# crlotwhite/pytorch_hmm

Hardware: AMD Instinct MI355X
Metric: frames/sec forward-backward+Viterbi, B=32 T=2000 N=128, 1/2/4/8 GPU (higher is better)
Workload: dtype f32; 1 GPU; HMMPyTorch forward_backward + viterbi_decode; batch_per_gpu=32, global_batch=32, seq_len=2000, num_states=128, transition=left_to_right(0.7), world_size_seen=1, parallelism=batch-sharded x1, streams=2, gather=False, hip_graph=False, step_pipelining=per-op streams, no per-step join, transition_plan=True, fb_kernel=chains + posterior followers in one launch, viterbi_kernel=chains + log leaders + decode followers in one launch

## Files before the change

pytorch_hmm_amd/csrc/recur.h:

```cpp
#pragma once
#include "band.h"
#include "common.h"
#include "logcr.h"
#include "post.h"

namespace hmm355 {

enum RecKind : int { kFbAlpha = 0, kFbBeta = 1, kVit = 2 };
typedef unsigned int u32x2_t __attribute__((__vector_size__(2 * sizeof(unsigned int))));

#ifndef HMM355_EMIS_AHEAD_ALPHA
#define HMM355_EMIS_AHEAD_ALPHA 1
#endif
#ifndef HMM355_EMIS_AHEAD_BETA
#define HMM355_EMIS_AHEAD_BETA 2
#endif
#ifndef HMM355_EMIS_AHEAD_VIT
#define HMM355_EMIS_AHEAD_VIT 2
#endif
constexpr int emis_ahead(int kind) {
  return kind == kFbAlpha ? HMM355_EMIS_AHEAD_ALPHA : kind == kFbBeta ? HMM355_EMIS_AHEAD_BETA : HMM355_EMIS_AHEAD_VIT;
}
#ifdef HMM355_RED_FORM
#define HMM355_RED_FORM_ALPHA HMM355_RED_FORM
#define HMM355_RED_FORM_BETA HMM355_RED_FORM
#define HMM355_RED_FORM_VIT HMM355_RED_FORM
#endif
#ifndef HMM355_RED_FORM_ALPHA
#define HMM355_RED_FORM_ALPHA 1
#endif
#ifndef HMM355_RED_FORM_BETA
#define HMM355_RED_FORM_BETA 3
#endif
#ifndef HMM355_RED_FORM_VIT
#define HMM355_RED_FORM_VIT 3
#endif
constexpr int red_form(int kind) {
  return kind == kFbAlpha ? HMM355_RED_FORM_ALPHA : kind == kFbBeta ? HMM355_RED_FORM_BETA : HMM355_RED_FORM_VIT;
}

constexpr int kStampWaves = 512 * 16;
static __device__ unsigned long long g_rec_stamps[kStamp ? kStampWaves * 8 : 1];
constexpr bool kStampItems = HMM355_STAMP > 1;

template <int NP>
struct RC {
  static constexpr int NW = NP / 16;
  static constexpr int NT = NW * kWave;
  static constexpr int NBLK = NP / 64;
  static constexpr int RING = 64;
  static constexpr int OFF_PART = 0;
  static constexpr int OFF_EMIS = OFF_PART + 2 * NP * 2;
  static constexpr int OFF_RING = OFF_EMIS + 3 * 16 * NP;
  static constexpr int OFF_SC = OFF_RING + RING * NP;
  static constexpr int OFF_M = OFF_SC + RING * 64;
  static constexpr int MRING = 128;
  static constexpr int OFF_LOGT = OFF_M + MRING;
  static constexpr int LDS_FLOATS = OFF_LOGT + 512;
  static_assert(LDS_FLOATS * 4 <= kExclusiveLds, "LDS layout too large");
  static constexpr int OFF_LEFT = LDS_FLOATS;
  static_assert((OFF_LEFT + 16) * 4 <= kExclusiveLds, "end-row LDS layout too large");
  static constexpr int PSR = 64;
  static constexpr int OFF_PSR = LDS_FLOATS;
  static_assert((OFF_PSR + PSR * NP / 4) * 4 <= kExclusiveLds, "fused Viterbi LDS layout too large");
};

template <int NP>
struct kRbHelpers {
  static constexpr int NH = NP <= 128 ? RC<NP>::NW / 2 : 0;
  static constexpr int NT = RC<NP>::NT + NH * kWave;
  static_assert(NH <= 8, "kProgSlots");
};
template <int NP>
constexpr int kFbNT = kRbHelpers<NP>::NT;

namespace red {
constexpr int kA = 1, kB = 2;
constexpr int stages(int F) { return 6 - (F & kA ? 1 : 0) - (F & kB ? 1 : 0); }
constexpr bool triple_at(int F, int L) { return (L == 0 && (F & kA)) || (L == 2 && (F & kB)); }
constexpr int level(int F, int S) {
  int L = 0;
  for (int s = 0; s < S; ++s) L += triple_at(F, L) ? 2 : 1;
  return L;
}
}
template <bool MAX, int SHR>
__device__ __forceinline__ float red_shr(float acc, float src) {
  const float o = __builtin_bit_cast(
      float, __builtin_amdgcn_update_dpp(0, __builtin_bit_cast(int, src), 0x110 + SHR, 0xF, 0xF, true));
  return MAX ? fmaxf(acc, o) : acc + o;
}
#define HMM355_RED_SHR2(VOL, OP)                                                            \
  asm VOL(OP " %0, %1, %0 row_shr:%2 row_mask:0xf bank_mask:0xf bound_ctrl:1\n\t"           \
          OP " %0, %1, %0 row_shr:%3 row_mask:0xf bank_mask:0xf bound_ctrl:1"               \
          : "+v"(acc) : "v"(src), "n"(S2), "n"(S3))
template <bool MAX, int S2, int S3, bool PIN>
__device__ __forceinline__ float red_shr2_asm(float acc, float src) {
  if constexpr (MAX && PIN) HMM355_RED_SHR2(volatile, "v_max_f32_dpp");
  else if constexpr (MAX) HMM355_RED_SHR2(, "v_max_f32_dpp");
  else if constexpr (PIN) HMM355_RED_SHR2(volatile, "v_add_f32_dpp");
  else HMM355_RED_SHR2(, "v_add_f32_dpp");
  return acc;
}
#undef HMM355_RED_SHR2
template <bool MAX, int S, int F = 0, bool PIN = false>
__device__ __forceinline__ float wave_red_level(float x) {
  constexpr int L = red::level(F, S);
  if constexpr (red::triple_at(F, L)) {
    constexpr int K = L == 0 ? 1 : 4;
    return red_shr2_asm<MAX, 2 * K, 3 * K, PIN>(red_shr<MAX, K>(x, x), x);
  } else {
    constexpr int CTRL = L == 0 ? 0xB1 : L == 1 ? 0x4E : L == 2 ? 0x124 : L == 3 ? 0x128 : L == 4 ? 0x142 : 0x143;
    const float o = __builtin_bit_cast(
        float, __builtin_amdgcn_update_dpp(0, __builtin_bit_cast(int, x), CTRL, 0xF, 0xF, L >= 4));
    return MAX ? fmaxf(x, o) : x + o;
  }
}
__device__ __forceinline__ float wave_lane63(float x) {
  return __builtin_bit_cast(float, __builtin_amdgcn_readlane(__builtin_bit_cast(int, x), 63));
}

template <int F = 0>
__device__ __forceinline__ float wave_sum_bcast(float x) {
  static_for<0, red::stages(F)>([&](auto S) { x = wave_red_level<false, decltype(S)::value, F>(x); });
  return wave_lane63(x);
}
template <int F = 0>
__device__ __forceinline__ float wave_max_bcast(float x) {
  static_for<0, red::stages(F)>([&](auto S) { x = wave_red_level<true, decltype(S)::value, F>(x); });
  return wave_lane63(x);
}

constexpr int fill_gaps(int F) { return red::stages(F) + 2; }
constexpr int fill_slots(int F, int G) { return G == fill_gaps(F) - 2 ? 1 : 2; }
constexpr int emis_wait_gap(int F) {
#ifdef HMM355_EMIS_WAIT_GAP
  return HMM355_EMIS_WAIT_GAP;
#else
  return F == 0 ? 4 : red::stages(F) - 1;
#endif
}
constexpr int fill_cnt(int G, int NU, int F = 0) {
  const int NG = fill_gaps(F);
  int rem = NU, all = 0;
  for (int i = 0; i < NG; ++i) all += fill_slots(F, i);
  for (int i = 0; i < NG; ++i) {
    const int g = i == 0 ? NG - 1 : i - 1;
    const int c = fill_slots(F, g) < rem ? fill_slots(F, g) : rem;
    if (g == G) return c + (G == NG - 1 && NU > all ? NU - all : 0);
    rem -= c;
  }
  return 0;
}
constexpr int fill_lo(int G, int NU, int F = 0) {
  int lo = 0;
  for (int g = 0; g < G; ++g) lo += fill_cnt(g, NU, F);
  return lo;
}
__device__ __forceinline__ void fill_pin(float& x) { asm volatile("" : "+v"(x)); }
template <bool MAX, int F = 0, typename FILL>
__device__ __forceinline__ float wave_red_fill(float x, FILL&& fill) {
  constexpr int NS = red::stages(F);
  static_for<0, NS>([&](auto S) {
    __builtin_amdgcn_sched_barrier(0);
    fill(S);
    __builtin_amdgcn_sched_barrier(0);
    x = wave_red_level<MAX, decltype(S)::value, F, true>(x);
    if constexpr (!red::triple_at(F, red::level(F, decltype(S)::value))) fill_pin(x);
  });
  __builtin_amdgcn_sched_barrier(0);
  fill(std::integral_constant<int, NS>{});
  __builtin_amdgcn_sched_barrier(0);
  x = wave_lane63(x);
  __builtin_amdgcn_sched_barrier(0);
  fill(std::integral_constant<int, NS + 1>{});
  __builtin_amdgcn_sched_barrier(0);
  return x;
}

#if HMM355_RED_PROBE
static __global__ void red_probe_kernel(const float* in, float* out, int n) {
  const int v = blockIdx.x * (blockDim.x / kWave) + threadIdx.x / kWave;
  if (v >= n) return;
  const float x = in[(size_t)v * kWave + (threadIdx.x & (kWave - 1))];
  static_for<0, 4>([&](auto F) {
    const float m = wave_max_bcast<decltype(F)::value>(x), s = wave_sum_bcast<decltype(F)::value>(x);
    if ((threadIdx.x & (kWave - 1)) == 0) {
      out[(size_t)v * 8 + decltype(F)::value] = m;
      out[(size_t)v * 8 + 4 + decltype(F)::value] = s;
    }
  });
}
#endif

template <int NB>
__device__ __forceinline__ void prods(const float (&p)[NB], const float (&e)[NB], float (&prod)[NB]) {
// ... 677 lines not shown
  constexpr bool FB = KIND != kVit;
  constexpr int NM = NP / 64;
  typedef float f2 __attribute__((ext_vector_type(2)));
  const int tid = threadIdx.x;
  if (tid >= C::NT) {
    rec_rb_helper<NP, KIND>(a, lds, b);
    return;
  }
  __builtin_amdgcn_s_setprio(2);
  const int w = tid >> 6, l = tid & 63, r = l >> 4, c = l & 15;
  const int g = 4 * w + r;
  const int x = c >> 2;
  const int o = 4 * g + x;
  const int T = a.T, N = a.N;
  float* ring = lds + C::OFF_RING;
  float* Pv = lds + C::OFF_PART;

  f2 Mk[4][NM][2];
#pragma unroll
  for (int k = 0; k < 4; ++k)
#pragma unroll
    for (int m = 0; m < NM; ++m)
#pragma unroll
      for (int e = 0; e < 4; ++e) {
        const int i = 64 * m + 4 * c + e, ok = 4 * g + (k ^ x);
        const bool in = i < N && ok < N;
        const size_t idx = in ? (KIND == kFbBeta ? (size_t)ok * N + i : (size_t)i * N + ok) : 0;
        const float v = a.mat[idx];
        Mk[k][m][e >> 1][e & 1] = FB ? __expf(in ? v : -INFINITY) : (in ? v : -INFINITY);
      }

  const int qend = T;
  const int nblocks = (qend + 15) / 16;
  {
    float er0[5];
    if (KIND == kVit) rec_logt_fill<NP>(lds, l);
    rec_load<NP, KIND>(a, b, 0, w, l, er0);
    rec_stage<NP, KIND>(a, lds, 0, w, l, er0);
  }
  lds_barrier();

  auto emis = [&](int rho, int idx) -> const float& { return rec_emis<NP>(lds, rho, idx); };
  const bool writer = (c & 3) == 0;
  {
    const float v0 = rec_row0<NP, KIND>(a, b, o, emis(0, o));
    if (writer) {
      ring[o] = v0;
      if (KIND == kFbBeta) Pv[o] = v0 * emis(0, o);
    }
  }
  lds_barrier();

  RecStamps stamps;
  stamps.begin();
  auto mark = [&](int k) { stamps.mark(k); };

  auto stepq = [&](int q) {
    if (kStamp) mark(3);
    const float* src = KIND == kFbBeta ? Pv + ((q - 1) & 1) * NP : ring + ((q - 1) & (C::RING - 1)) * NP;
    float eo = emis(q, o);
    f2 yin[NM][2];
#pragma unroll
    for (int m = 0; m < NM; ++m) {
      const float4 v4 = *reinterpret_cast<const float4*>(src + 64 * m + 4 * c);
      yin[m][0] = f2{v4.x, v4.y};
      yin[m][1] = f2{v4.z, v4.w};
    }
    keep(eo);
    if (kStamp) { keep(yin[0][0]); mark(0); }
    float s0, s1, s2, s3;
    float cs = 0.f;
    if (FB) {
      f2 acc[4];
#pragma unroll
      for (int k = 0; k < 4; ++k) acc[k] = f2{0.f, 0.f};
      f2 ysum = f2{0.f, 0.f};
#pragma unroll
      for (int m = 0; m < NM; ++m)
#pragma unroll
        for (int p = 0; p < 2; ++p) {
#pragma unroll
          for (int k = 0; k < 4; ++k) acc[k] = __builtin_elementwise_fma(yin[m][p], Mk[k][m][p], acc[k]);
          ysum += yin[m][p];
        }
      float cx = ysum.x + ysum.y;
      s0 = acc[0].x + acc[0].y; s1 = acc[1].x + acc[1].y;
      s2 = acc[2].x + acc[2].y; s3 = acc[3].x + acc[3].y;
      red4_add_with_c(s0, s1, s2, s3, cx);
      cs = cx;
    } else {
      float mx[4];
#pragma unroll
      for (int m = 0; m < NM; ++m)
#pragma unroll
        for (int p = 0; p < 2; ++p) {
          f2 t[4];
#pragma unroll
          for (int k = 0; k < 4; ++k) t[k] = yin[m][p] + Mk[k][m][p];
#pragma unroll
          for (int k = 0; k < 4; ++k)
            mx[k] = (m == 0 && p == 0) ? fmaxf(t[k].x, t[k].y) : fmaxf(fmaxf(mx[k], t[k].x), t[k].y);
        }
      s0 = mx[0]; s1 = mx[1]; s2 = mx[2]; s3 = mx[3];
      red4_max(s0, s1, s2, s3);
    }
    if (kStamp) { keep(s0); mark(1); }
    float val, pval = 0.f;
    if (FB) {
      const float scale = __builtin_amdgcn_rcpf(cs);
      if (w == 0) lds[C::OFF_SC + 64 * ((q - 1) & (C::RING - 1))] = cs;
      val = KIND == kFbAlpha ? s0 * (scale * eo) : s0 * scale;
      if (KIND == kFbBeta) pval = val * eo;
    } else {
      val = s0 + eo;
    }
    ring[(q & (C::RING - 1)) * NP + o] = val;
    if (KIND == kFbBeta) Pv[(q & 1) * NP + o] = pval;
    if (kStamp) { mark(2); ++stamps.steps; }
    step_barrier();
  };
  auto run_block = [&](int kb) {
    const int q0 = kb * 16 < 1 ? 1 : kb * 16;
    const int q1 = (kb + 1) * 16 < qend ? (kb + 1) * 16 : qend;
    if (q0 == kb * 16 && q1 == q0 + 16) {
#pragma unroll
      for (int i = 0; i < 16; ++i) stepq(kb * 16 + i);
    } else {
      for (int q = q0; q < q1; ++q) stepq(q);
    }
  };
  for (int k = 0; k < nblocks; ++k) run_block(k);
  stamps.finish(blockIdx.x * C::NW + w);
  if (KIND == kFbAlpha && a.loglik && w == C::NW - 1) {
    float ys = 0.f;
#pragma unroll
    for (int m = 0; m < NM; ++m) ys += ring[((T - 1) & (C::RING - 1)) * NP + 64 * m + l];
    rec_keep_c_last<NP>(lds, T, ys);
  }
  lds_barrier();
}

constexpr bool win_term_shifted(int n, int NB, int TD0) { return (n % NB + TD0 + n / NB + 4 * NB) / NB != 4; }
constexpr int win_term_src(int n, int NB, int TD0) { return n % NB + TD0 + n / NB + 4 * NB; }
constexpr int win_shift_term(int m, int NB, int NWIN, int TD0) {
  int c = 0;
  for (int n = NB; n < NWIN; ++n) {
    bool first = win_term_shifted(n, NB, TD0);
    for (int p = NB; p < n; ++p) first = first && win_term_src(p, NB, TD0) != win_term_src(n, NB, TD0);
    if (first && c++ == m) return n;
  }
  return c;
}

template <int NP, int KIND, int WP, int TD0 = 0, int TW = 0, int EA = emis_ahead(KIND)>
__device__ __forceinline__ void band_chain(const RecArgs& a, float* lds, int b, const BandDesc* __restrict__ d) {
  using C = RC<NP>;
  constexpr int NB = C::NBLK;
  constexpr bool FB = KIND != kVit;
  constexpr bool FUSE = KIND == kVit && kVitFused<NP>;
  const int l = threadIdx.x & 63;
  const int T = a.T, N = a.N;
  const int nblocks = (T + 15) / 16;
  constexpr int WW = TW > 0 ? TW : WP;
  int lo[NB];
  float wv[NB][WW], fl[NB];
#pragma unroll
  for (int j = 0; j < NB; ++j) {
    const int s = NB * l + j;
    lo[j] = KIND == kFbBeta ? d->rlo[s] : d->clo[s];
#pragma unroll
    for (int k = 0; k < WW; ++k) {
      if (TW > 0)
        wv[j][k] = KIND == kVit ? d->tL[s][k] : (KIND == kFbAlpha ? d->tD[s][k] : d->tR[s][k]);
      else
        wv[j][k] = KIND == kVit ? d->cL[s][k] : (KIND == kFbAlpha ? d->cD[s][k] : d->rD[s][k]);
    }
    fl[j] = KIND == kVit ? d->rfl[s] : d->afl[s];
  }
  const bool uafl = d->uafl != 0;
  const float afl0 = d->afl[0];
  auto erow = [&](int rho) { return lds + C::OFF_EMIS + (((rho >> 4) % 3) * 16 + (rho & 15)) * NP + NB * l; };
  auto ld = [&](const float* p, float(&v)[NB]) {
    if constexpr (NB == 1) v[0] = p[0];
    else if constexpr (NB == 2) { const float2 t = *reinterpret_cast<const float2*>(p); v[0] = t.x; v[1] = t.y; }
    else { const float4 t = *reinterpret_cast<const float4*>(p); v[0] = t.x; v[1] = t.y; v[2] = t.z; v[3] = t.w; }
  };
  auto pin_all = [&](float(&v)[NB]) {
    if constexpr (NB == 1) asm volatile("" : "+v"(v[0]));
    else if constexpr (NB == 2) asm volatile("" : "+v"(v[0]), "+v"(v[1]));
    else asm volatile("" : "+v"(v[0]), "+v"(v[1]), "+v"(v[2]), "+v"(v[3]));
  };
  auto st = [&](float* p, const float(&v)[NB]) {
    if constexpr (NB == 1) p[0] = v[0];
    else if constexpr (NB == 2) *reinterpret_cast<float2*>(p) = make_float2(v[0], v[1]);
    else *reinterpret_cast<float4*>(p) = make_float4(v[0], v[1], v[2], v[3]);
  };
  float y[NB];
  {
    float e0[NB];
    ld(erow(0), e0);
#pragma unroll
    for (int j = 0; j < NB; ++j) y[j] = rec_row0<NP, KIND>(a, b, NB * l + j, e0[j]);
  }
  float* ybuf = lds + C::OFF_PART;
  constexpr int EL = KIND == kFbBeta ? 1 : 0;
  float en[EA][NB];
  constexpr bool kSumFirst = NB == 4 || (NB == 2 && TW >= 2 && TD0 >= 0);
  float pp[NB], ee[NB];
  float gprev = -INFINITY;

  auto at = [&](const float(&v)[NB], int j, int dd) -> float {
    const int t = j + dd + 4 * NB;
    const int qq = t / NB - 4, jj = t % NB;
    const int x = __builtin_bit_cast(int, v[jj]);
    if (qq == 0) return v[jj];
    if (qq == -1) return __builtin_bit_cast(float, __builtin_amdgcn_update_dpp(0, x, 0x138, 0xF, 0xF, true));
    if (qq == 1) return __builtin_bit_cast(float, __builtin_amdgcn_update_dpp(0, x, 0x130, 0xF, 0xF, true));
    if (qq == -2) {
      const int t1 = __builtin_amdgcn_update_dpp(0, x, 0x138, 0xF, 0xF, true);
      return __builtin_bit_cast(float, __builtin_amdgcn_update_dpp(0, t1, 0x138, 0xF, 0xF, true));
    }
    const int t1 = __builtin_amdgcn_update_dpp(0, x, 0x130, 0xF, 0xF, true);
    return __builtin_bit_cast(float, __builtin_amdgcn_update_dpp(0, t1, 0x130, 0xF, 0xF, true));
  };

  auto step = [&](int q, int jj, bool no_read, auto UA, auto FP, auto RL, auto ES, auto PW, float* row, const float* enext,
                  float& blk, auto wlane) {
    constexpr bool FILLED = KIND != kFbAlpha;
    constexpr int RF = red_form(KIND);
    constexpr bool LW = TW == 0;
    constexpr bool WFILL = !(KIND == kFbAlpha && !decltype(UA)::value);
    constexpr int NWIN = NB * WW;
    constexpr bool SPLIT = FILLED && FB && !LW;
    constexpr int NSH = SPLIT ? win_shift_term(-1, NB, NWIN, TD0) : 0;
    constexpr int O_LD = 1, O_ST2 = O_LD + (LW ? NWIN : 0), O_EN = O_ST2 + (LW && KIND == kFbBeta ? 1 : 0);
    constexpr int O_T = O_EN + 1, O_SH = O_T + (SPLIT ? NB : 0), NU = O_T + (WFILL ? NWIN + NSH : 0);
    float eo[NB];
#pragma unroll
    for (int j = 0; j < NB; ++j) eo[j] = en[decltype(ES)::value][j];
    float acc[NB], src[NB], wl[NB][WW], tv[NB][WW], sh[5 * NB];
    float cs = 0.f, scale = 1.f;
    const float* wsrc = KIND == kFbBeta ? ybuf + ((q - 1) & 1) * NP : row;
    auto term = [&](int n) {
      const int j = LW ? n / WW : n % NB, k = LW ? n % WW : n / NB;
      float v;
      if constexpr (LW) v = wl[j][k];
      else v = (SPLIT && k > 0 && win_term_shifted(n, NB, TD0)) ? sh[win_term_src(n, NB, TD0) - 2 * NB] : at(src, j, TD0 + k);
      if (FB) {
        if (WFILL && k == 0) {
#pragma clang fp contract(off)
          acc[j] = v * wv[j][k];
        } else {
          acc[j] = fmaf(v, wv[j][k], acc[j]);
        }
      } else {
        tv[j][k] = v + wv[j][k];
      }
    };
    auto shift = [&](int m) {
      const int n = win_shift_term(m, NB, NWIN, TD0);
      float& s = sh[win_term_src(n, NB, TD0) - 2 * NB];
      s = at(src, n % NB, TD0 + n / NB);
      fill_pin(s);
    };
    auto unit = [&](auto I) {
      constexpr int i = decltype(I)::value;
      if constexpr (i == 0) {
        if (LW && KIND == kFbBeta) st(ybuf + ((q - 1) & 1) * NP + NB * l, src);
        else st(row + NB * l, y);
      } else if constexpr (i < O_ST2) {
        wl[(i - O_LD) / WW][(i - O_LD) % WW] = wsrc[lo[(i - O_LD) / WW] + (i - O_LD) % WW];
      } else if constexpr (i < O_EN) {
        st(row + NB * l, y);
      } else if constexpr (i == O_EN) {
        if constexpr (!(kAbl & abl::kBandEmisReg)) {
          if (!no_read) ld(enext, en[decltype(ES)::value]);
        }
      } else if constexpr (i < O_SH) {
        term(i - O_T);
      } else if constexpr (i < O_SH + NSH) {
        shift(i - O_SH);
      } else {
        term(i - O_T - NSH);
      }
    };
    auto fill = [&](auto G) {
      static_for<fill_lo(decltype(G)::value, NU, RF), fill_lo(decltype(G)::value + 1, NU, RF)>(unit);
      if constexpr (decltype(PW)::value && decltype(G)::value == emis_wait_gap(RF) && !(kAbl & abl::kBandEmisReg))
        pin_all(en[EA - 1 - decltype(ES)::value]);
    };
    auto reduce = [&](auto MAXOP, float t) -> float {
      if constexpr (kAbl & abl::kBandNoReduce) {
        static_for<0, NU>(unit);
        return __builtin_bit_cast(float, __builtin_amdgcn_readfirstlane(__builtin_bit_cast(int, t)));
      } else if constexpr (!FILLED) {
        static_for<0, NU>(unit);
        return decltype(MAXOP)::value ? wave_max_bcast<RF>(t) : wave_sum_bcast<RF>(t);
      } else if constexpr (decltype(MAXOP)::value && (kAbl & abl::kBandReducePrev)) {
        const float r = wave_red_fill<true, RF>(gprev, fill);
        gprev = t;
        return r;
      } else {
        return wave_red_fill<decltype(MAXOP)::value, RF>(t, fill);
      }
    };
    if (KIND == kFbBeta) {
      prods<NB>(y, eo, src);
      const float t = prod_sum<NB, kSumFirst || decltype(RL)::value>(y, eo, src);
#pragma unroll
      for (int j = 0; j < NB; ++j) acc[j] = 0.f;
      cs = reduce(std::false_type{}, t);
    } else if (KIND == kFbAlpha) {
#pragma unroll
      for (int j = 0; j < NB; ++j) src[j] = y[j];
      float t;
      if constexpr (decltype(FP)::value) t = prod_sum<NB, kSumFirst>(pp, ee, y);
      else t = plain_sum<NB>(y);
      if constexpr (decltype(UA)::value) {
#pragma unroll
        for (int j = 0; j < NB; ++j) acc[j] = 0.f;
        cs = reduce(std::false_type{}, t);
      } else {
        float tw = 0.f;
#pragma unroll
        for (int j = 0; j < NB; ++j) tw = fmaf(y[j], fl[j], tw);
        cs = reduce(std::false_type{}, t);
        tw = wave_sum_bcast<RF>(tw);
#pragma unroll
        for (int j = 0; j < NB; ++j) acc[j] = tw;
      }
    } else {
      float g = -INFINITY;
#pragma unroll
      for (int j = 0; j < NB; ++j) { src[j] = y[j]; g = fmaxf(g, y[j] + fl[j]); }
      const float M = reduce(std::true_type{}, g);
      if constexpr (FUSE) wlane(blk, M);
#pragma unroll
      for (int j = 0; j < NB; ++j) acc[j] = M;
    }
    if (FB) {
      scale = __builtin_amdgcn_rcpf(cs);
      wlane(blk, cs);
    }
    if constexpr (!WFILL) {
      static_for<0, NWIN>([&](auto I) { term(decltype(I)::value); });
    } else if constexpr (!FB) {
#pragma unroll
      for (int n = 0; n < NWIN; ++n) {
        const int j = LW ? n / WW : n % NB, k = LW ? n % WW : n / NB;
        acc[j] = fmaxf(acc[j], tv[j][k]);
      }
    }
    if constexpr (KIND == kFbAlpha) {
#pragma unroll
      for (int j = 0; j < NB; ++j) {
        if constexpr (decltype(UA)::value) { pp[j] = fmaf(acc[j], scale, afl0); ee[j] = eo[j]; }
        else { pp[j] = acc[j]; ee[j] = scale * eo[j]; }
      }
      prods<NB>(pp, ee, y);
    }
#pragma unroll
    for (int j = 0; j < NB; ++j) {
      if (KIND == kFbAlpha) continue;
      if (KIND == kFbBeta) {
        y[j] = fmaf(acc[j], scale, fl[j]);
      } else {
        y[j] = acc[j] + eo[j];
      }
    }
  };

  unsigned long long st_bar = 0, st_t0 = 0;
  long long rt0 = 0;
  if (kStamp) { st_t0 = stamp(); rt0 = __builtin_amdgcn_s_memrealtime(); }
  auto run_blocks = [&](auto UA) {
    for (int kb = 0; kb < nblocks; ++kb) {
      const int q0 = kb * 16 < 1 ? 1 : kb * 16;
      const int q1 = (kb + 1) * 16 < T ? (kb + 1) * 16 : T;
      if (q0 < q1) ld(erow(q0 - EL), en[0]);
      float* rbase = lds + C::OFF_RING + ((16 * kb) & (C::RING - 1)) * NP;
      float* rwrap = lds + C::OFF_RING + ((16 * kb - 1) & (C::RING - 1)) * NP;
      const float* ebase = lds + C::OFF_EMIS + ((kb % 3) * 16 + 1 - EL) * NP + NB * l;
      float blk = 0.f;
      if (q0 == kb * 16 && q1 == kb * 16 + 16) {
        static_for<1, EA>([&](auto K) { ld(ebase + (decltype(K)::value - 1) * NP, en[decltype(K)::value]); });
        static_for<0, 16>([&](auto JJ) {
          constexpr int jj = decltype(JJ)::value;
          step(kb * 16 + jj, jj, jj + EA > 15, UA, std::bool_constant<(jj > 0)>{}, std::bool_constant<(jj == 0)>{},
               std::integral_constant<int, jj % EA>{}, std::bool_constant<(EA == 2 && KIND != kFbAlpha && jj < 15)>{},
               jj == 0 ? rwrap : rbase + (jj - 1) * NP, ebase + (jj + EA - 1) * NP, blk,
               [](float& d, float v) { writelane_c<jj>(d, v); });
        });
        if constexpr (FB || FUSE) {
          if (l < 16) lds[C::OFF_SC + 64 * ((16 * kb + l - 1) & (C::RING - 1))] = blk;
        }
      } else {
        for (int q = q0; q < q1; ++q) {
          const int jj = q - kb * 16;
          float* sc = lds + C::OFF_SC + 64 * ((q - 1) & (C::RING - 1));
          step(q, jj, q + 1 == q1, UA, std::false_type{}, std::true_type{}, std::integral_constant<int, 0>{}, std::false_type{},
               jj == 0 ? rwrap : rbase + (jj - 1) * NP, ebase + jj * NP, blk,
               [sc](float&, float v) { *sc = v; });
        }
      }
      unsigned long long sb = 0;
      if (kStamp) sb = stamp();
      if (!(kAbl & abl::kBandNoBlockBarrier)) lds_barrier();
      if (kStamp) st_bar += stamp() - sb;
    }
  };
  if constexpr (KIND == kFbAlpha) {
    if (uafl) run_blocks(std::true_type{});
    else run_blocks(std::false_type{});
  } else {
    run_blocks(std::false_type{});
  }
  if (kStamp && l == 0) {
    const unsigned long long t1 = stamp();
    const long long rt1 = __builtin_amdgcn_s_memrealtime();
    unsigned long long* o8 = g_rec_stamps + ((size_t)blockIdx.x * 16 % kStampWaves) * 8;
    o8[0] = (unsigned long long)rt0; o8[1] = (unsigned long long)rt1; o8[3] = st_bar;
    o8[4] = T; o8[5] = t1 - st_t0; o8[6] = t1 - st_t0; o8[7] = (unsigned long long)(rt1 - rt0);
  }
  float* row = lds + C::OFF_RING + ((T - 1) & (C::RING - 1)) * NP;
  st(row + NB * l, y);
  if (KIND == kFbAlpha && a.loglik) {
    float t = 0.f;
#pragma unroll
    for (int j = 0; j < NB; ++j) t += y[j];
    rec_keep_c_last<NP>(lds, T, t);
  }
  lds_barrier();
}

template <int NP, int KIND, int WP, int TD0 = 0, int TW = 0>
__device__ __forceinline__ void rec_band(const RecArgs& a, float* lds, int b, const BandDesc* __restrict__ d) {
  using C = RC<NP>;
  constexpr int NB = C::NBLK;
  constexpr bool FUSE = KIND == kVit && kVitFused<NP>;
  constexpr bool WIDE = FUSE;
  constexpr bool FBW = KIND != kVit;
  constexpr int NWB = kFbNT<NP> / kWave;
  constexpr int NH = WIDE ? 6 : FBW ? (NWB / 4) * 3 + (NWB % 4 > 1 ? NWB % 4 - 1 : 0)
                                    : ((KIND == kVit && C::NW >= 8) ? 4 : 3);
  constexpr int HV = (C::NW + NH - 1) / NH;
  const int tid = threadIdx.x;
  const int w = tid >> 6, l = tid & 63;
  const int grp = (w >> 3) * 3 + (w & 3) - 1;
  const bool stager = WIDE ? ((w & 4) == 0 && (w & 3) != 0) : FBW ? (w & 3) != 0 : (w > 0 && w <= NH);
  const bool psiw = WIDE && (w & 4) != 0 && (w & 3) != 0;
  const int hi = WIDE ? grp : FBW ? (w >> 2) * 3 + (w & 3) - 1 : w - 1;
  auto vw_of = [&](int h) -> int { return hi + h * NH; };
  constexpr bool FB = KIND != kVit;
  if (w != 0 && !stager && !psiw) return;
  const int T = a.T, N = a.N;
  const int nblocks = (T + 15) / 16;
  double base = (KIND == kFbBeta && a.bscale) ? (double)a.bscale[b] : 0.0;

  float er0[HV][5], er1[HV][5], er2[HV][5];
  if (stager) {
    if (KIND == kVit) rec_logt_fill<NP>(lds, l);
#pragma unroll
    for (int h = 0; h < HV; ++h) {
      const int vw = vw_of(h);
      if (vw < C::NW) {
        float er[5];
        rec_load<NP, KIND>(a, b, 0, vw, l, er);
        rec_stage<NP, KIND, FUSE>(a, lds, 0, vw, l, er);
        if (nblocks > 1) rec_load<NP, KIND>(a, b, 1, vw, l, er1[h]);
        if (nblocks > 2) rec_load<NP, KIND>(a, b, 2, vw, l, er2[h]);
      }
    }
  }
  lds_barrier();

  if (w == 0) {
    band_chain<NP, KIND, WP, TD0, TW>(a, lds, b, d);
    return;
  }
    constexpr int PWN = TW > 0 ? TW : WP;
    [[maybe_unused]] float prf[NB];
    [[maybe_unused]] int plo[NB];
    [[maybe_unused]] float pcl[NB][PWN];
    if constexpr (FUSE) {
#pragma unroll
      for (int j = 0; j < NB; ++j) {
        const int o = NB * l + j;
        prf[j] = o < N ? d->rfl[o] : -INFINITY;
        plo[j] = TW > 0 ? o + TD0 : d->clo[o];
#pragma unroll
        for (int kk = 0; kk < PWN; ++kk) {
          const int i = plo[j] + kk;
          pcl[j][kk] = (i >= 0 && i < N && o < N) ? (TW > 0 ? d->tL[o][kk] : d->cL[o][kk]) : -INFINITY;
        }
      }
#pragma unroll
      for (int j = 0; j < NB; ++j) {
        keep(prf[j]);
        keep(plo[j]);
#pragma unroll
        for (int kk = 0; kk < PWN; ++kk) keep(pcl[j][kk]);
      }
    }
    auto psi_rows = [&](int bk) {
      if constexpr (FUSE) {
        if (bk < 0 || (kAbl & abl::kNoPsiRows)) return;
        constexpr int NPW = WIDE ? 6 : 3, PR = (16 + NPW - 1) / NPW;
        const int hw = grp;
#pragma unroll
        for (int m = 0; m < PR; ++m) {
          const int r = hw + NPW * m;
          int t = 16 * bk + (r < 16 ? r : 15);
          t = t < T ? t : T - 1;
          const int rho = (t - 1) & (C::RING - 1);
          const float* drow = lds + C::OFF_RING + rho * NP;
          float yv[NB], xw[NB][PWN];
          if constexpr (NB == 2) {
            const float2 v2 = *reinterpret_cast<const float2*>(drow + NB * l);
            yv[0] = v2.x; yv[1] = v2.y;
          } else {
            const float4 v4 = *reinterpret_cast<const float4*>(drow + NB * l);
            yv[0] = v4.x; yv[1] = v4.y; yv[2] = v4.z; yv[3] = v4.w;
          }
          const float M = lds[C::OFF_SC + 64 * rho];
#pragma unroll
          for (int j = 0; j < NB; ++j)
#pragma unroll
            for (int kk = 0; kk < PWN; ++kk) {
              const int i = plo[j] + kk;
              xw[j][kk] = drow[i < 0 ? 0 : (i < NP ? i : NP - 1)];
            }
          int i1 = 0x7fffffff;
#pragma unroll
          for (int j = 0; j < NB; ++j) {
            const float g = yv[j] + prf[j];
            const unsigned long long hit = __ballot(g == M);
            const int c = NB * (__ffsll((long long)hit) - 1) + j;
            i1 = (hit && c < i1) ? c : i1;
          }
          unsigned pk = 0;
#pragma unroll
          for (int j = 0; j < NB; ++j) {
            float v = M, val[PWN];
#pragma unroll
            for (int kk = 0; kk < PWN; ++kk) {
              val[kk] = xw[j][kk] + pcl[j][kk];
              v = fmaxf(v, val[kk]);
            }
            int arg = M == v ? i1 : 0x7fffffff;
#pragma unroll
            for (int kk = 0; kk < PWN; ++kk)
              if (val[kk] == v && plo[j] + kk < arg) arg = plo[j] + kk;
            arg = (NB * l + j < N && t > 0) ? arg : 0;
            pk |= (unsigned)arg << (8 * j);
          }
          if (r < 16 && 16 * bk + r < T) {
            uint8_t* ldst = reinterpret_cast<uint8_t*>(lds + C::OFF_PSR) + (t & (C::PSR - 1)) * NP + NB * l;
            if constexpr (NB == 2) *reinterpret_cast<uint16_t*>(ldst) = (uint16_t)pk;
            else *reinterpret_cast<uint32_t*>(ldst) = pk;
          }
        }
      }
    };
    const bool pubon = a.pub != nullptr;
    int* const pubp = pubon ? a.pub + (FB ? 2 * b + (KIND == kFbBeta) : b) * kPubStride : nullptr;
    [[maybe_unused]] const __amdgpu_buffer_rsrc_t psi_rs =
        FUSE ? make_rsrc(a.psi + (size_t)b * T * NP, (size_t)T * NP) : make_rsrc(a.obs, 0);
    [[maybe_unused]] auto psi_copy = [&](int bk) {
      if constexpr (FUSE) {
        constexpr int PER = NP / 16;
        const int hidx = (NH - 1 - hi) * 64 + l;
        const int r = hidx / PER, pc = hidx % PER;
        const int t = 16 * bk + r;
        const u32x4_t v = *reinterpret_cast<const u32x4_t*>(reinterpret_cast<const uint8_t*>(lds + C::OFF_PSR) +
                                                            (t & (C::PSR - 1)) * NP + 16 * pc);
        if (bk >= 0 && hidx < 16 * PER && t < T)
          __builtin_amdgcn_raw_buffer_store_b128(v, psi_rs, t * NP + 16 * pc, 0, (kFAbl & fabl::kPlainStores) ? 0 : kAuxSc1);
      }
    };
    const bool lpon = KIND == kVit && a.lready;
    const __amdgpu_buffer_rsrc_t lp_rs =
        make_rsrc(lpon ? static_cast<const void*>(a.lready + b * kPubStride) : static_cast<const void*>(a.obs), lpon ? 8 : 0);
    auto lp_count = [&](const u32x2_t& v) -> int {
      const unsigned lo = __builtin_amdgcn_readfirstlane(v[0]), hi32 = __builtin_amdgcn_readfirstlane(v[1]);
      const unsigned c = lo ^ count_mix(a.token);
      return (hi32 == a.token && c <= (unsigned)nblocks) ? (int)c : 0;
    };
    unsigned long long hs_work = 0, hs_wait = 0, hs_item[4] = {0, 0, 0, 0};
    constexpr int KL = NP / 64;
    constexpr int RE = (16 * kEndBlocks + NH - 1) / NH;
    [[maybe_unused]] float epr[RE][KL];
    [[maybe_unused]] int eok = 0;
    const bool endson = FB && stager && pubon && (a.ends & kEndsOn) && a.prow && a.post;
    const int qend0 = 16 * (nblocks - kEndBlocks);
    auto end_row = [&](int m, int& q) -> bool {
      q = qend0 + hi + NH * m;
      return q < T;
    };
    [[maybe_unused]] auto end_load = [&]() {
      if constexpr (FB) {
        const int* ppub = a.pub + (2 * b + (KIND == kFbAlpha)) * kPubStride;
        const int cnt = __builtin_amdgcn_readfirstlane(poll_count(ppub, a.token, nblocks + 1));
        const bool counted = cnt > nblocks || 16 * cnt >= T - qend0;
        int leftmask = 0;
#pragma unroll
        for (int m = 0; m < RE; ++m) {
          int q;
          const bool live = end_row(m, q);
          const bool ok = counted && !((a.ends & kEndsOddLeft) && ((q >> 4) & 1));
          eok |= (int)ok << m;
          if (live && !ok) leftmask |= 1 << (nblocks - 1 - (q >> 4));
          int tq = live ? rec_tau<KIND>(q, T) : 0;
          asm volatile("" : "+v"(tq) : "s"(cnt));
          post_row_load<KL>(make_rsrc(a.prow + (size_t)b * T * NP, (size_t)T * NP * 4), tq, l, epr[m]);
        }
        if (l == 0) reinterpret_cast<int*>(lds + C::OFF_LEFT)[hi] = leftmask;
      }
    };
    [[maybe_unused]] auto end_post = [&]() {
      if constexpr (FB) {
        const bool endvec = N == NP && (reinterpret_cast<uintptr_t>(a.post) % (4 * KL)) == 0;
#pragma unroll
        for (int m = 0; m < RE; ++m) {
          int q;
          const bool on = end_row(m, q) && ((eok >> m) & 1);
          const int tq = on ? rec_tau<KIND>(q, T) : 0;
          float own[KL];
          const float* rp = lds + C::OFF_RING + (q & (C::RING - 1)) * NP + KL * l;
          if constexpr (KL == 1) {
            own[0] = rp[0];
// ... 237 lines not shown
```

Before: 401.3 million frames/s.

## Software-pipeline band chain across block edges with barrier inside the block

Adds an edge-pipelined variant of the band recursion loop, enabled by default. Full 16-step blocks no longer wait at the block boundary: emissions for the next block are prefetched from the next staging slot and the LDS barrier is issued mid-block, after step 15-EA. Ring and scale indices are kept as incrementally advanced offsets instead of being recomputed. The goal is to hide barrier and emission-load latency at block boundaries on the serial chain wave. The cost is more code and a reliance on followers keeping pace with the earlier barrier point. It also adds extra timing-stamp counters under the stamp build flag.

```diff
diff --git a/pytorch_hmm_amd/csrc/recur.h b/pytorch_hmm_amd/csrc/recur.h
--- a/pytorch_hmm_amd/csrc/recur.h
+++ b/pytorch_hmm_amd/csrc/recur.h
@@ -21,6 +21,10 @@
 constexpr int emis_ahead(int kind) {
   return kind == kFbAlpha ? HMM355_EMIS_AHEAD_ALPHA : kind == kFbBeta ? HMM355_EMIS_AHEAD_BETA : HMM355_EMIS_AHEAD_VIT;
 }
+#ifndef HMM355_BLOCK_EDGE
+#define HMM355_BLOCK_EDGE 1
+#endif
+constexpr bool kBlockEdge = HMM355_BLOCK_EDGE;
 #ifdef HMM355_RED_FORM
 #define HMM355_RED_FORM_ALPHA HMM355_RED_FORM
 #define HMM355_RED_FORM_BETA HMM355_RED_FORM
@@ -42,6 +46,10 @@
 constexpr int kStampWaves = 512 * 16;
 static __device__ unsigned long long g_rec_stamps[kStamp ? kStampWaves * 8 : 1];
 constexpr bool kStampItems = HMM355_STAMP > 1;
+#ifndef HMM355_STAMP_BAR
+#define HMM355_STAMP_BAR 1
+#endif
+constexpr bool kStampBar = HMM355_STAMP_BAR;
 
 template <int NP>
 struct RC {
@@ -1025,7 +1033,7 @@
   return c;
 }
 
-template <int NP, int KIND, int WP, int TD0 = 0, int TW = 0, int EA = emis_ahead(KIND)>
+template <int NP, int KIND, int WP, int TD0 = 0, int TW = 0, int EA = emis_ahead(KIND), bool EDGE = false>
 __device__ __forceinline__ void band_chain(const RecArgs& a, float* lds, int b, const BandDesc* __restrict__ d) {
   using C = RC<NP>;
   constexpr int NB = C::NBLK;
@@ -1243,10 +1251,17 @@
     }
   };
 
-  unsigned long long st_bar = 0, st_t0 = 0;
+  unsigned long long st_bar = 0, st_t0 = 0, st_steady = 0, st_edge = 0, st_nsteady = 0, st_nedge = 0, st_bar_in = 0;
   long long rt0 = 0;
   if (kStamp) { st_t0 = stamp(); rt0 = __builtin_amdgcn_s_memrealtime(); }
+  auto block_barrier = [&]() {
+    unsigned long long sb = 0;
+    if (kStamp && kStampBar) sb = stamp();
+    if (!(kAbl & abl::kBandNoBlockBarrier)) lds_barrier();
+    if (kStamp && kStampBar) st_bar += stamp() - sb;
+  };
   auto run_blocks = [&](auto UA) {
+    unsigned long long s15 = 0;
     for (int kb = 0; kb < nblocks; ++kb) {
       const int q0 = kb * 16 < 1 ? 1 : kb * 16;
       const int q1 = (kb + 1) * 16 < T ? (kb + 1) * 16 : T;
@@ -1259,11 +1274,21 @@
         static_for<1, EA>([&](auto K) { ld(ebase + (decltype(K)::value - 1) * NP, en[decltype(K)::value]); });
         static_for<0, 16>([&](auto JJ) {
           constexpr int jj = decltype(JJ)::value;
+          if (kStamp && jj == 1) {
+            const unsigned long long s1 = stamp();
+            if (s15) { st_edge += s1 - s15; ++st_nedge; }
+            s15 = s1;
+          }
           step(kb * 16 + jj, jj, jj + EA > 15, UA, std::bool_constant<(jj > 0)>{}, std::bool_constant<(jj == 0)>{},
                std::integral_constant<int, jj % EA>{}, std::bool_constant<(EA == 2 && KIND != kFbAlpha && jj < 15)>{},
                jj == 0 ? rwrap : rbase + (jj - 1) * NP, ebase + (jj + EA - 1) * NP, blk,
                [](float& d, float v) { writelane_c<jj>(d, v); });
         });
+        if (kStamp) {
+          const unsigned long long t = stamp();
+          st_steady += t - s15; ++st_nsteady;
+          s15 = t;
+        }
         if constexpr (FB || FUSE) {
           if (l < 16) lds[C::OFF_SC + 64 * ((16 * kb + l - 1) & (C::RING - 1))] = blk;
         }
@@ -1276,17 +1301,81 @@
                [sc](float&, float v) { *sc = v; });
         }
       }
-      unsigned long long sb = 0;
-      if (kStamp) sb = stamp();
-      if (!(kAbl & abl::kBandNoBlockBarrier)) lds_barrier();
-      if (kStamp) st_bar += stamp() - sb;
-    }
+      block_barrier();
+    }
+  };
+  auto run_edge = [&](auto UA) {
+    auto rolled = [&](int kb, int q0, int q1) {
+      if (q0 < q1) ld(erow(q0 - EL), en[0]);
+      float* rbase = lds + C::OFF_RING + ((16 * kb) & (C::RING - 1)) * NP;
+      float* rwrap = lds + C::OFF_RING + ((16 * kb - 1) & (C::RING - 1)) * NP;
+      const float* ebase = lds + C::OFF_EMIS + ((kb % 3) * 16 + 1 - EL) * NP + NB * l;
+      float none = 0.f;
+      for (int q = q0; q < q1; ++q) {
+        const int jj = q - kb * 16;
+        float* sc = lds + C::OFF_SC + 64 * ((q - 1) & (C::RING - 1));
+        step(q, jj, q + 1 == q1, UA, std::false_type{}, std::true_type{}, std::integral_constant<int, 0>{}, std::false_type{},
+             jj == 0 ? rwrap : rbase + (jj - 1) * NP, ebase + jj * NP, none,
+             [sc](float&, float v) { *sc = v; });
+      }
+      block_barrier();
+    };
+    rolled(0, 1, T < 16 ? T : 16);
+    const int nfull = T / 16 - 1;
+    if (nfull > 0) {
+      static_for<0, EA>([&](auto K) { ld(erow(16 + decltype(K)::value - EL), en[decltype(K)::value]); });
+      int es = 16 * NP, rb = 16 * NP;
+      int scw = 64 * ((15 + (l & 15)) & (C::RING - 1)) + (l >> 4);
+      float blk = 0.f;
+      unsigned long long s15 = 0;
+      for (int kb = 1; kb <= nfull; ++kb) {
+        const int esn = es == 32 * NP ? 0 : es + 16 * NP;
+        float* rbase = lds + C::OFF_RING + rb;
+        float* rwrap = lds + C::OFF_RING + ((rb - NP) & (C::RING * NP - 1));
+        const float* ebase = lds + C::OFF_EMIS + es + (1 - EL) * NP + NB * l;
+        const float* nbase = lds + C::OFF_EMIS + esn + NB * l;
+        static_for<0, 16>([&](auto JJ) {
+          constexpr int jj = decltype(JJ)::value;
+          constexpr int p = jj + EA - EL;
+          if (kStamp && jj == 1) {
+            const unsigned long long s1 = stamp();
+            if (s15) { st_edge += s1 - s15; ++st_nedge; }
+            s15 = s1;
+          }
+          step(kb * 16 + jj, jj, false, UA, std::bool_constant<(jj > 0)>{}, std::bool_constant<(jj == 0)>{},
+               std::integral_constant<int, jj % EA>{}, std::bool_constant<(EA == 2 && KIND != kFbAlpha)>{},
+               jj == 0 ? rwrap : rbase + (jj - 1) * NP, p < 16 ? ebase + (jj + EA - 1) * NP : nbase + (p - 16) * NP, blk,
+               [](float& d, float v) { writelane_c<jj>(d, v); });
+          if constexpr (jj == 15 - EA) {
+            const unsigned long long b0 = st_bar;
+            block_barrier();
+            st_bar_in += st_bar - b0;
+          }
+        });
+        if (kStamp) {
+          const unsigned long long t = stamp();
+          st_steady += t - s15; ++st_nsteady;
+          s15 = t;
+        }
+        if constexpr (FB || FUSE) {
+          lds[C::OFF_SC + scw] = blk;
+          scw = (scw + 16 * 64) & (C::RING * 64 - 1);
+        }
+        es = esn;
+        rb = (rb + 16 * NP) & (C::RING * NP - 1);
+      }
+    }
+    if (T > 16 && (T & 15)) rolled(T / 16, T & ~15, T);
+  };
+  auto run = [&](auto UA) {
+    if constexpr (EDGE) run_edge(UA);
+    else run_blocks(UA);
   };
   if constexpr (KIND == kFbAlpha) {
-    if (uafl) run_blocks(std::true_type{});
-    else run_blocks(std::false_type{});
+    if (uafl) run(std::true_type{});
+    else run(std::false_type{});
   } else {
-    run_blocks(std::false_type{});
+    run(std::false_type{});
   }
   if (kStamp && l == 0) {
     const unsigned long long t1 = stamp();
@@ -1294,6 +1383,8 @@
     unsigned long long* o8 = g_rec_stamps + ((size_t)blockIdx.x * 16 % kStampWaves) * 8;
     o8[0] = (unsigned long long)rt0; o8[1] = (unsigned long long)rt1; o8[3] = st_bar;
     o8[4] = T; o8[5] = t1 - st_t0; o8[6] = t1 - st_t0; o8[7] = (unsigned long long)(rt1 - rt0);
+    unsigned long long* e8 = g_rec_stamps + (((size_t)blockIdx.x * 16 + 4) % kStampWaves) * 8;
+    e8[0] = st_steady; e8[1] = st_nsteady; e8[2] = st_edge; e8[3] = st_nedge; e8[4] = st_bar_in;
   }
   float* row = lds + C::OFF_RING + ((T - 1) & (C::RING - 1)) * NP;
   st(row + NB * l, y);
@@ -1348,7 +1439,7 @@
   lds_barrier();
 
   if (w == 0) {
-    band_chain<NP, KIND, WP, TD0, TW>(a, lds, b, d);
+    band_chain<NP, KIND, WP, TD0, TW, emis_ahead(KIND), kBlockEdge>(a, lds, b, d);
     return;
   }
     constexpr int PWN = TW > 0 ? TW : WP;
```

New measurement: 421.3 million frames/s, median of 6. 5.0% higher.
